# JvanZyl1/PSSO-SAC-for-powered-descent

Hardware: AMD Instinct MI355X
Metric: env-steps/sec at 65 536 parallel envs; achieved HBM GB/s vs peak (higher is better)
Workload: dtype f64; 1 GPU; c3: 65536 envs/GPU, landing_burn_pure_throttle, rtd_rl reward, wind (percentile profile drawn per reset + VK gusts below 15 km) + tilt, auto-reset, uniform random actions; synchronized starts, 640 untimed burn-in + 5 warmup steps; envs_per_gpu=65536, global_envs=65536, parallelism=env-shard x1

## Files before the change

include/pdenv.h:

```cpp
#ifndef PDENV_H
#define PDENV_H
#include <stddef.h>
#include <stdint.h>

#ifdef __cplusplus
extern "C" {
#endif

#define PD_ABI_VERSION 11
#define PD_MAX_PTS 256
#define PD_MAX_COLS 5
#define PD_MAX_TAB 64
#define PD_MAX_WIND 16
#define PD_N_WIND_PROFILES 50
#define PD_N_STATE 11
#define PD_N_INFO 49
#define PD_ACTOR_PARAMS_PURE_THROTTLE 249
#define PD_ACTOR_PARAMS_LANDING_BURN 372

typedef enum { PD_OK = 0, PD_ERR_INVALID = 1, PD_ERR_HIP = 2, PD_ERR_NOMEM = 3, PD_ERR_UNSUPPORTED = 4 } pd_status;
typedef enum {
    PD_PHASE_PURE_THROTTLE = 0, PD_PHASE_LANDING_BURN = 1, PD_PHASE_PCONTROL = 2,
    PD_PHASE_BALLISTIC_ARC = 3, PD_PHASE_FLIP_OVER = 4, PD_PHASE_SUBSONIC = 5, PD_PHASE_SUPERSONIC = 6,
    PD_PHASE_LANDING_BURN_ACS = 7
} pd_phase;
typedef enum { PD_RTD_RL = 0, PD_RTD_PSO = 1, PD_RTD_NONE = 2 } pd_rtd;
typedef enum { PD_F64 = 0, PD_F32 = 1 } pd_precision;
typedef enum { PD_INTEG_REFERENCE = 0, PD_INTEG_RK4 = 1 } pd_integrator;
typedef enum {
    PD_TABLES_NO_CELL_PIECES = 1,
    PD_TABLES_NO_FINE_INDEX = 2,
    PD_TABLES_EXACT_ATMOSPHERE = 4,
    PD_TABLES_VERBOSE = 8
} pd_table_flags;

typedef struct {
    int32_t n_cols, n_pts;
    double col_aoa[PD_MAX_COLS];
    int32_t col_start[PD_MAX_COLS], col_len[PD_MAX_COLS];
    double mach[PD_MAX_PTS];
    double coef[PD_MAX_PTS];
} pd_aero_table;

typedef struct {
    double thrust_per_engine, nozzle_exit_pressure, nozzle_exit_area, v_exhaust;
    int32_t n_engines_gimballed, pad0;
    double grid_fin_area, d_base_grid_fin, rocket_radius, frontal_area, m_prop0, C_gust_x, C_gust_y;
    double h_ox, h_f, m_ox, m_f, h_lower, m_dry, x_dry, I_dry, engine_height, cop;
// ... 145 lines not shown
pd_status pd_set_gload_window(pd_env* env, const void* vprev, const void* window, const uint8_t* len,
                              void* stream);
pd_status pd_get_gload_window(pd_env* env, void* vprev, void* window, uint8_t* len, uint8_t* head, void* stream);
pd_status pd_set_wind_sigmas(pd_env* env, const double* sig, void* stream);
pd_status pd_get_wind_state(pd_env* env, void* filters, void* sigmas, uint8_t* profile, void* stream);
pd_status pd_set_wind_state(pd_env* env, const void* filters, const void* sigmas, const uint8_t* profile, void* stream);
pd_status pd_get_counters(pd_env* env, uint32_t* episode, uint32_t* step, int8_t* trunc_id, void* stream);
pd_status pd_set_counters(pd_env* env, const uint32_t* episode, const uint32_t* step, const int8_t* trunc_id,
                          void* stream);
size_t pd_checkpoint_size(const pd_env* env);
pd_status pd_checkpoint_save(pd_env* env, void* blob, void* stream);
pd_status pd_checkpoint_load(pd_env* env, const void* blob, void* stream);
pd_status pd_counters(pd_env* env, int64_t* rbf_misses, int64_t* table_entries_cd,
                      int64_t* table_entries_cl, int64_t* nan_events);
pd_status pd_atmosphere(pd_env* env, const void* altitude, void* out, int64_t n, void* stream);
#define PD_N_STATS 48
pd_status pd_stats(pd_env* env, int64_t* out, int32_t n);
pd_status pd_count_work(pd_env* env, int32_t enable);
pd_status pd_cell_piece_info(const pd_params* params, int32_t table, int64_t piece, double* out, int32_t n_out);
pd_status pd_atm_table(const pd_params* params, int32_t precision, const double* alt, int64_t n_alt,
                       double* atm_out, double* max_rel);
int pd_obs_dim(const pd_env* env);
int pd_action_dim(const pd_env* env);

#ifdef __cplusplus
}
#endif
#endif
```

psso-sac-for-powered-descent_amd/csrc/pd_physics.h:

```cpp
#pragma once
#include "pd_common.h"

namespace pd {

template <typename R> struct Cst;
template <> struct Cst<double> {
    static constexpr double deg2rad = kDeg2Rad, rad2deg = kRad2Deg, pi = kPi, two_pi = 2 * kPi;
    static constexpr double inf = __builtin_huge_val();
};
template <> struct Cst<float> {
    static constexpr float deg2rad = (float)kDeg2Rad, rad2deg = (float)kRad2Deg, pi = (float)kPi,
                           two_pi = (float)(2 * kPi);
    static constexpr float inf = __builtin_huge_valf();
};

template <typename R> constexpr R veltkamp_c() { return sizeof(R) == 8 ? R(134217729.0) : R(4097.0f); }
template <typename R> constexpr bool one_step_ok(R b, R rb) {
    const R p = b * rb;
    const R C = veltkamp_c<R>();
    const R tb = C * b, bh = tb - (tb - b), bl = b - bh;
    const R tr = C * rb, rh = tr - (tr - rb), rl = rb - rh;
    const R lo = ((bh * rh - p) + bh * rl + bl * rh) + bl * rl;
    const R eps = (p - R(1)) + lo;
    const R lim = sizeof(R) == 8 ? R(0.99 * 0x1p-54) : R(0.99f * 0x1p-25f);
// ... 293 lines not shown
            int j = kind == 5 ? 4 + k : (kind == 6 ? 4 + k : (k < 6 ? k : k + 1));
            put(k, (R)(float)((R)(float)s[j] / P.norm_ph[k]));
        }
    }
}
template <typename R>
__device__ __forceinline__ void obs_write(DP<R>& P, int kind, const R* s, R* out, uint32_t idx) {
    const int d = obs_dim(kind);
    PD_AS1 char* o = (PD_AS1 char*)(uint64_t)out;
    obs_eval<R>(P, kind, s, [&](int k, R v) {
        *(PD_AS1 R*)(o + (uint32_t)(idx * (uint32_t)(d * sizeof(R)) + k * (uint32_t)sizeof(R))) = v;
    });
}

template <typename R>
__device__ __forceinline__ R grid_fin_ca(DP<R>& P, const R* sx, const R* sy, R mach, const uint16_t* lb = nullptr,
                                         const R* slope = nullptr) {
    if (mach < P.ca_min_mach) return P.ca_min_val;
    int n = P.ca_n;
    int lo = 0, hi = n;
    if (lb != nullptr && mach >= R(0) && mach < R(10)) {
        int b = (int)(mach * R(6.4));
        b = b > 63 ? 63 : b;
        const uint32_t rg = lb[b];
        lo = (int)(rg & 0xffu); hi = (int)(rg >> 8);
    }
    while (lo < hi) { int mid = (lo + hi) >> 1; if (sx[mid] < mach) lo = mid + 1; else hi = mid; }
    int idx = lo < 1 ? 1 : (lo > n - 1 ? n - 1 : lo);
    R xl = sx[idx - 1], yl = sy[idx - 1];
    const R sl = slope ? slope[idx] : (sy[idx] - yl) / (sx[idx] - xl);
    return sl * (mach - xl) + yl;
}

template <typename R>
__device__ __forceinline__ R np_interp(const R* x, const R* y, int n, R v, const R* slope = nullptr) {
    if (v < x[0]) return y[0];
    if (v >= x[n - 1]) return y[n - 1];
    int lo = 0, hi = n;
    while (lo < hi) { int mid = (lo + hi) >> 1; if (x[mid] <= v) lo = mid + 1; else hi = mid; }
    int j = lo - 1;
    if (x[j] == v) return y[j];
    const R sl = slope ? slope[j] : (y[j + 1] - y[j]) / (x[j + 1] - x[j]);
    return sl * (v - x[j]) + y[j];
}

template <typename R>
__device__ __forceinline__ R grid_fin_cn_alpha(DP<R>& P, const R* sx, const R* sy, R mach, const R* slope = nullptr) {
    if (mach < P.cn_min_mach) return P.cn_min_val;
    if (mach <= P.cn_max_mach) return np_interp(sx, sy, P.cn_n, mach, slope);
    return P.cn_max_val + P.cn_slope * (mach - P.cn_max_mach);
}

template <typename R> struct RbfCache {
    unsigned long long key;
    int slot;
};

template <typename R>
// ... 65 lines not shown
```

psso-sac-for-powered-descent_amd/csrc/pd_step.h:

```cpp
#pragma once
#include <hip/hip_runtime.h>

#include <cstring>

#include "../../include/pdenv.h"
#include "pd_physics.h"
#include "pd_sac_mlp.h"

namespace pd {

constexpr int kBlock = 256;
constexpr int kStepBlock = 256;
constexpr int kScratch = kSys * kSys + kSys + 3 * kNbr + kPay;
constexpr int kPendingCap = 4096;
constexpr int kSolveSlots = 1024;
constexpr int kGridExact = 1 << 30;
constexpr int kGridRefine = 1 << 29;
constexpr int kGridBisect = 1 << 28;
constexpr int kGridPiece = 1 << 27;
constexpr uint32_t kFinePiece = 1u << 30;
constexpr uint32_t kFineBisect = 1u << 29;
constexpr uint32_t kFineRefined = 1u << 28;
constexpr uint32_t kFineIndex = kFineRefined - 1u;

// ... 2 lines not shown
constexpr int kCellExact = 4;
constexpr int kCellKey = kCellCoef + 3 * kCellExact;
constexpr int kCellStride = (kCellKey + 2) & ~1;
constexpr int kCellKeyF = (kCellKey + 1) & ~1;
constexpr int kCellStrideF = (kCellKeyF + 2 + 3) & ~3;
template <typename R> constexpr int cell_stride() { return sizeof(R) == 8 ? kCellStride : kCellStrideF; }
template <typename R> constexpr int cell_key() { return sizeof(R) == 8 ? kCellKey : kCellKeyF; }

struct GridBisect {
    double nx, ny, c, tau;
    unsigned long long key_a, key_b;
    int slot_a, slot_b;
    int piece_a, piece_b;
};
constexpr int kGridSub = 8;
constexpr int kStats = 48;

enum Stat {
    kStMisses = 0, kStNan = 1, kStInsCd = 2, kStInsCl = 3,
    kStStamp = 8,
    kStDropped = 16,
    kStWork = 32,
    kStGust = kStWork + 0,
    kStResets = kStWork + 1,
    kStQLine = kStWork + 2,
    kStQVerify = kStWork + 3,
    kStQTaylor = kStWork + 4,
    kStQBal = kStWork + 5,
    kStQMiss = kStWork + 6,
    kStBalRounds = kStWork + 7,
    kStQRefined = kStWork + 8,
    kStQBisect = kStWork + 9,
    kStWRefined = kStWork + 10,
    kStWBisect = kStWork + 11,
    kStQCell = kStWork + 12,
    kStWMixed = kStWork + 13,
    kNWork = 14
};

struct WaveCount {
    uint32_t* w;
    __device__ __forceinline__ void add(int k, bool pred) {
        if (w) {
            const uint32_t v = (uint32_t)__popcll(__ballot(pred));
            if (__lane_id() == 0) w[k] += v;
        }
    }
    __device__ __forceinline__ void add_n(int k, uint32_t v) {
        if (w && __lane_id() == 0) w[k] += v;
    }
};

template <typename R> struct LineLds {
    R bp[4][kLineMax];
    int slot[4][kLineMax + 1];
    unsigned long long key[4][kLineMax + 1];
    R a[4];
    int nbp[4];
    int tay_off[4];
    uint16_t lb[4][kLineBuckets];
};

template <typename R, bool WIND> struct alignas(16) StepStatic {
    alignas(16) R tab[1024];
// ... 79 lines not shown
        for (uint32_t p = 0; p <= mask; ++p) {
            const unsigned long long k = keys[h];
            if (k == key) { slot = -1; break; }
            if (k == kEmptyKey) { slot = (int)h; break; }
            h = (h + 1) & mask;
        }
        if (slot >= 0 && stats[kStInsCd + table] * 2 + 2 > (1ull << lc)) slot = -1;
        if (slot < 0) continue;
        stats[kStInsCd + table] += 1;
        keys[slot] = key;
        pay_store<R>(ppay + e * kPay, (table ? pay_cl : pay_cd) + (int64_t)slot * pay_stride<R>());
    }
    *count = 0;
}

template <typename R> struct StepArgs {
    uint64_t P;
    EnvBufs<R> b;
    Pending pend;
    int64_t n;
    uint64_t env_offset;
    uint32_t seed_lo, seed_hi;
    int act_f64, auto_reset, stochastic, fixed_prof, use_tilt;
    double tilt_sigma;
    const void* actions;
    R* obs; R* reward; uint8_t* done; uint8_t* trunc; int8_t* trunc_id;
    const double* noise;
    R* info;
    uint64_t info_mask;
    int info_nsel;
// ... 37 lines not shown
```

psso-sac-for-powered-descent_amd/csrc/pd_step_impl.h:

```cpp
#pragma once
#include "pd_envdev.h"

namespace pd {

__device__ __forceinline__ int dpp_swap1(int v) { return __builtin_amdgcn_mov_dpp(v, 0xB1, 0xF, 0xF, false); }
__device__ __forceinline__ float pair_swap(float v) { return __int_as_float(dpp_swap1(__float_as_int(v))); }
__device__ __forceinline__ double pair_swap(double v) {
    const uint64_t b = (uint64_t)__double_as_longlong(v);
    const uint32_t lo = (uint32_t)dpp_swap1((int)(uint32_t)b), hi = (uint32_t)dpp_swap1((int)(uint32_t)(b >> 32));
    return __longlong_as_double((long long)(((uint64_t)hi << 32) | lo));
}

template <int LPE, typename R>
__device__ __forceinline__ void sincos_pair(R x0, R x1, int role, R& s0, R& c0, R& s1, R& c1) {
    if constexpr (LPE >= 2) {
        const bool odd = role & 1;
        R s, c;
        pd_sincos<R>(odd ? x1 : x0, s, c);
        const R so = pair_swap(s), co = pair_swap(c);
        s0 = odd ? so : s; c0 = odd ? co : c;
        s1 = odd ? s : so; c1 = odd ? c : co;
    } else {
        pd_sincos<R>(x0, s0, c0);
        pd_sincos<R>(x1, s1, c1);
// ... 820 lines not shown
    if constexpr (OSPLIT) gather(ys, y, OS);
    else {
#pragma unroll
        for (int j = 0; j < OUT; ++j) y[j] = ys[j];
    }
}

#ifdef PD_STAMP
#define PD_T(v) const unsigned long long v = __builtin_amdgcn_s_memtime()
#define PD_ACC(k, d) acc_[k] += (d)
#else
#define PD_T(v)
#define PD_ACC(k, d)
#endif

template <typename R, bool WIND, int EPB, bool BAL = false> struct StepLds : StepStatic<R, WIND> {
    R gwin[10][EPB];
    uint32_t work[kStepBlock / 64][kNWork];
    double wnx[WIND ? 2 : 1][WIND ? kStepBlock : 1];
    BalLds<R> bal[BAL ? kStepBlock / 64 : 1];
    TabView<R> tdesc[2];
};

template <typename R>
__device__ __forceinline__ TabView<R> tab_view_lds(const TabView<R>* d, int table) { return d[table]; }
template <typename R>
__device__ __forceinline__ TabView<R> tab_view(DP<R>& P, const R* tab, int table) {
    TabView<R> t;
    t.smach = tab + (table ? 512 : 0);
    t.start = table ? &P.cl_start[0] : &P.cd_start[0];
    t.n = table ? &P.cl_len[0] : &P.cd_len[0];
    t.aoa = table ? &P.cl_aoa[0] : &P.cd_aoa[0];
    t.keys = gbl(table ? P.keys_cl : P.keys_cd);
// ... 12 lines not shown
    t.grid_na = P.grid_na[table];
    t.grid_a0 = P.grid_a0[table];
    t.grid_inv_da = P.grid_inv_da[table];
    t.grid_inv_dm = P.grid_inv_dm[table];
    return t;
}

template <typename R, int PHASE, int RTD, bool WIND, int LPE, int POL = 0, bool RK4 = false, bool CNT = false,
          bool SAC = false, bool ROLL = false>
__global__ __launch_bounds__(kStepBlock) __attribute__((amdgpu_waves_per_eu(2))) void k_step(StepArgs<R> a_) {
    SA<R>& a = kargs<R>();
    static_assert(sizeof(a_) > 0);
    static_assert(!ROLL || (SAC && LPE == 16 && !POL && !RK4 && !CNT && RTD == 0 && PHASE <= 1),
                  "ROLL: the SAC kernel of the RL landing burns at 16 lanes per env");
    constexpr int EPB = kStepBlock / LPE;
    __shared__ StepLds<R, WIND, EPB, LPE == 2> L;
#ifdef PD_STAMP
    unsigned long long acc_[17] = {};
#endif
    PD_T(t_start);
    int64_t n_act = a.n;
    constexpr bool kRefill = POL && !WIND;
    int64_t ring_pos0 = 0;
    if constexpr (SAC) { if (a.ring_state) ring_pos0 = (int64_t)__atomic_load_n(a.ring_state, __ATOMIC_RELAXED); }
    if constexpr (POL) {
        if (blockIdx.x == 0 && threadIdx.x == 0) *a.cnt_zero = 0u;
        if (kRefill && a.refill) n_act = a.refill_slots;
        if (a.use_list) {
            n_act = (int64_t)*a.cnt_in;
            if ((int64_t)blockIdx.x * EPB >= n_act) return;
        }
// ... 18 lines not shown
    const int le = (int)threadIdx.x / LPE;
    uint32_t ui = (uint32_t)i;
    bool live = valid;
    if constexpr (POL) {
        if (!a.use_list) live = live && ev(a.b.fin, ui) == 0;
    }
    if constexpr (ROLL) live = live && ev(a.b.fin, ui) == 0;
    constexpr int nparts = LPE >= 2 ? LPE / 2 : 1;
    const int my_table = LPE >= 2 ? role / nparts : 0;
    const int part = LPE >= 2 ? role % nparts : 0;
    const int gbase = (int)__lane_id() & ~(LPE - 1);
    uint64_t g = a.env_offset + (uint64_t)i;

    EnvRegs<R> e;
    RbfCache<R> cA, cB;
    auto load_env = [&]() {
        DP<R>& P = *params<R>(a.P);
#pragma unroll
        for (int k = 0; k < 11; ++k) e.s[k] = valid ? ldv(a.b.st + (k) * N, ui) : P.state0[k];
        e.vprev = valid ? ldv(a.b.vprev, ui) : sqrt(e.s[2] * e.s[2] + e.s[3] * e.s[3]);
        e.glen = valid ? (int)ldv(a.b.glen, ui) : 0;
        e.ghead = valid ? (int)ldv(a.b.ghead, ui) : 0;
#pragma unroll
        for (int k = 0; k < 10; ++k) L.gwin[k][le] = valid ? ldv(a.b.gwin + (k) * N, ui) : R(0);
        e.act0 = R(0); e.act1 = R(0); e.act2 = R(0);
        if constexpr (PHASE == 1 || PHASE == 2) e.act0 = valid ? ldv(a.b.act, ui) : R(0);
        if constexpr (PHASE == 1) {
            e.act1 = valid ? ldv(a.b.act + N, ui) : R(0);
            e.act2 = valid ? ldv(a.b.act + (2) * N, ui) : R(0);
        }
        e.fu0 = R(0); e.fu1 = R(0); e.fv0 = R(0); e.fv1 = R(0); e.sgu = R(0); e.sgv = R(0); e.prof = 0;
        if constexpr (WIND) {
            if (valid) {
                e.fu0 = ldv(a.b.wind, ui); e.fu1 = ldv(a.b.wind + N, ui);
                e.fv0 = ldv(a.b.wind + (2) * N, ui); e.fv1 = ldv(a.b.wind + (3) * N, ui);
                e.sgu = ldv(a.b.wind + (4) * N, ui); e.sgv = ldv(a.b.wind + (5) * N, ui);
                e.prof = ldv(a.b.wprof, ui);
            }
        }
        e.ep = valid ? ldv(a.b.epi, ui) : 0u;
        e.ts = valid ? ldv(a.b.tstep, ui) : 0u;
        e.tid = valid ? (int)ldv(a.b.tid, ui) : 0;
        cA.key = valid ? ldv(a.b.key + (my_table) * N, ui) : (my_table ? P.init_key_cl : P.init_key_cd);
        cA.slot = valid ? ldv(a.b.slot + (my_table) * N, ui) : -1;
        if constexpr (LPE == 1) { cB.key = valid ? ldv(a.b.key + N, ui) : P.init_key_cl; cB.slot = valid ? ldv(a.b.slot + N, ui) : -1; }
        else { cB.key = 0; cB.slot = -1; }
    };
    load_env();
    constexpr int kImg = (int)(sizeof(StepStatic<R, WIND>) / 16);
    constexpr int kLog = (int)(sizeof(LogTableD) / 16);
    constexpr int kPer = (kImg + kLog + kStepBlock - 1) / kStepBlock;
    using V4 = __attribute__((ext_vector_type(4))) unsigned int;
    V4 stg[kPer];
    {
        DP<R>& P = *params<R>(a.P);
        const PD_AS1 V4* img = (const PD_AS1 V4*)P.stage_img;
        const PD_AS1 V4* lgt = (const PD_AS1 V4*)(uint64_t)&P.logtab_d.cell[0];
#pragma unroll
        for (int k = 0; k < kPer; ++k) {
// ... 16 lines not shown
                if (a.sac_heads_out && e0 + e < a.n) a.sac_heads_out[(e0 + e) * 2 * A2 + o] = v;
            };
            if (H == 128) sac_mlp_tile<128>(a.sac_mlp, a.n, e0, s_mlp, put);
            else sac_mlp_tile<256>(a.sac_mlp, a.n, e0, s_mlp, put);
            __syncthreads();
        }
    }
    {
        DP<R>& P = *params<R>(a.P);
#pragma unroll
        for (int k = 0; k < kPer; ++k) {
            const int t = threadIdx.x + k * kStepBlock;
            if (t < kImg) ((V4*)static_cast<StepStatic<R, WIND>*>(&L))[t] = stg[k];
            else if (t < kImg + kLog) ((V4*)s_logtab)[t - kImg] = stg[k];
        }
        if (threadIdx.x < (kStepBlock / 64) * kNWork) (&L.work[0][0])[threadIdx.x] = 0u;
        if (threadIdx.x < 2) L.tdesc[threadIdx.x] = tab_view<R>(P, L.tab, (int)threadIdx.x);
    }
    __syncthreads();
    PD_T(t_staged);
    PD_ACC(0, t_staged - t_start);
    if constexpr (POL) {
        if (!a.use_list && __ballot(live) == 0) return;
    }
    const int aux = PHASE == 2 ? params<R>(a.P)->phase : PHASE;
    const bool ascent = PHASE == 2 && (aux == PD_PHASE_SUBSONIC || aux == PD_PHASE_SUPERSONIC);
    constexpr int A = PHASE == 0 ? 1 : (PHASE == 1 ? 4 : 2);
    const int AD = PHASE == 2 ? (ascent ? 2 : 1) : A;
    static_assert(!RK4 || (PHASE == 0 && !WIND && !POL), "RK4: pure throttle, no wind, no policy");
    constexpr int NSUB = RK4 ? 40 : (PHASE == 2 ? 1 : 4);
    constexpr bool kAtmTab = sizeof(R) == 4 || !WIND;
    constexpr bool kPcs = !WIND && !RK4 && LPE <= 8 && (PHASE == 0 || (PHASE == 1 && !SAC));
    const R dt = RK4 ? R(0.01) : (PHASE == 0 ? R(0.025) : (PHASE == 1 ? R(0.1) : (R)a.dt_aux));
    const R dt_act = PHASE == 2 ? dt : R(0.025);
    PD_T(t_loaded);
    PD_ACC(1, t_loaded - t_staged);

    auto store_all = [&]() {
    uint32_t uo = ui;
    asm volatile("" : "+v"(uo));
    if (live) {
        const uint32_t ui = uo;
#pragma unroll
        for (int k = 0; k < 11; ++k)
            if (k % LPE == role) ev(a.b.st + (k) * N, ui) = e.s[k];
// ... 43 lines not shown
        if (a.roll_steps) ev(a.roll_steps, uo) = (int32_t)steps;
        if (a.roll_done) ev(a.roll_done, uo) = (uint8_t)dn_;
        if (a.roll_tid) ev(a.roll_tid, uo) = (int8_t)id_;
        if (fin_) ev(a.b.fin, uo) = 1;
    };
    WaveCount wc{CNT ? L.work[threadIdx.x >> 6] : nullptr};
    R k_rho = R(0), k_patm = R(0), k_asnd = R(0);
    double k_speed = 0.0;
    bool k_have = false;
    using RS = double;
    RS xs[sizeof(R) == 8 ? 1 : 11];
    auto SV = [&](int k) -> RS& {
        if constexpr (sizeof(R) == 8) return e.s[k];
        else return xs[k];
    };
#pragma unroll 1
    for (int f = 0; f < nf; ++f) {
    SA<R>& a = kargs<R>();
    const size_t fo = (size_t)f * (size_t)N;
    float uf[A];
    double ud[A];
#pragma unroll
    for (int k = 0; k < A; ++k) { uf[k] = 0.f; ud[k] = 0.0; }
    if constexpr (ROLL) {
        if (role == 0) {
            DP<R>& Q = *params<R>(a.P);
            constexpr int ok = PHASE == 0 ? 0 : 3;
            obs_eval<R>(Q, ok, e.s, [&](int k, R v) { s_obs[le * obs_dim(ok) + k] = (float)v; });
        }
        if (!__syncthreads_or(live ? 1 : 0)) break;
// ... 42 lines not shown
            float xk = m;
            if (a.sac_eps || a.sac_draw) {
                float ls = mlp ? s_sach[le * 16 + 8 + k] : ldv(a.sac_logstd + k, ui * a.sac_hs);
                ls = ls < a.sac_lo ? a.sac_lo : (ls > a.sac_hi ? a.sac_hi : ls);
                const float sd = expf(ls);
                const float ek = a.sac_draw ? ed[k] : ldv(a.sac_eps + k, ui * AD);
                xk = m + sd * ek;
                if (a.sac_eps_out && role == 0 && live) ev(a.sac_eps_out + k, ui * AD) = ek;
            }
            uf[k] = tanhf(xk) * a.sac_max;
            if (a.sac_act && role == 0 && live) ev(a.sac_act + k, ui * AD) = uf[k];
            if constexpr (ROLL) {
                if (a.roll_act && role == 0 && live)
                    ev(a.roll_act + (size_t)(a.roll_t0 + f) * (size_t)N * (size_t)AD + k, ui * AD) = uf[k];
            }
        }
    } else if (a.act_f64) {
#pragma unroll
        for (int k = 0; k < A; ++k) if (k < AD) ud[k] = ldv((const double*)a.actions + fo * AD + k, ui * AD);
    } else {
#pragma unroll
        for (int k = 0; k < A; ++k) if (k < AD) uf[k] = ldv((const float*)a.actions + fo * AD + k, ui * AD);
    }
    constexpr int kObsKind = RTD == 1 ? (PHASE == 0 ? 1 : 2) : (PHASE == 0 ? 0 : (PHASE == 1 ? 3 : -1));
    uint32_t srow = ui;
    if (SAC && a.ring_state) {
        const int64_t rp = ring_pos0 + (int64_t)i;
        srow = (uint32_t)(rp >= a.ring_cap ? rp - a.ring_cap : rp);
    }
    if (SAC && a.slab && role == 0 && live) {
// ... 20 lines not shown

    bool wpre = false;
    RS rkb[8], rka[8];
    if constexpr (sizeof(R) == 4) {
#pragma unroll
        for (int k = 0; k < 11; ++k) xs[k] = (RS)e.s[k];
    }
    const RS dts = RK4 ? 0.01 : (PHASE == 0 ? 0.025 : (PHASE == 1 ? 0.1 : a.dt_aux));
#pragma unroll 1
    for (int sub = 0; sub < NSUB; ++sub) {
        PD_T(t_sub);
        const int stage = RK4 ? (sub & 3) : 0;
        SA<R>& a = kargs<R>();
        DP<R>& P = *params<R>(a.P);
        const bool tap_sub = tap && sub == NSUB - 1;
        RS x = SV(0), y = SV(1), vx = SV(2), vy = SV(3), th = SV(4), thd = SV(5), ga = SV(6), al = SV(7);
        RS m = SV(8), mp = SV(9);
        if constexpr (WIND) wc.add(kStGust - kStWork, role == 0 && live && a.stochastic && y < P.vk_y_threshold);
        R rho, patm, asnd;
        RS speed;
        if (RK4 ? (sub == 0 && k_have) : k_have) { rho = k_rho; patm = k_patm; asnd = k_asnd; speed = k_speed; }
        else {
            atmosphere<R, kAtmTab>(P, L.isa, (R)y, rho, patm, asnd);
            speed = sqrt(vx * vx + vy * vy);
        }
        const R spR = (R)speed;
        R mach = R(0);
        if (asnd != R(0)) { R mr = spR / asnd; mach = (R(10) < mr) ? R(10) : mr; }
        const R ae = (R)((vy < RS(0)) ? ga - th - Cst<RS>::pi : al);
        R ug = R(0), vg = R(0);
        auto wind_block = [&]() {
            if constexpr (WIND) {
                const R* walt = L.walt + e.prof * 16;
                const R* wsp = L.wsp + e.prof * 16;
                R km = PD_DIVC(R, (R)y, 1000);
                int wn = P.wind_n[e.prof];
                ug = np_interp<R>(walt, wsp, wn, km);
                const bool gust = y < P.vk_y_threshold && a.stochastic;
                if (gust) {
                    double w0 = 0.0, w1 = 0.0;
                    const double* lic = (const double*)(uint64_t)&P.logtab.invc[0];
                    const double* llc = (const double*)(uint64_t)&P.logtab.logc[0];
                    bool drawn = false;
                    if (a.noise) { w0 = ev(a.noise + 2 * sub, ui * 8); w1 = ev(a.noise + 2 * sub + 1, ui * 8); drawn = true; }
                    else if constexpr (LPE >= 2 && NSUB == 4) {
                        if ((sub & 1) == 0) {
                            const int odd = role & 1;
                            u32x4 r = philox_k({(uint32_t)g, (uint32_t)(g >> 32) ^ e.ep, e.ts, kTagWindSub + (uint32_t)(sub + odd)},
                                             a.seed_lo, a.seed_hi);
                            double z0, z1;
                            gauss_pair(r, lic, llc, z0, z1);
                            const double o0 = pair_swap(z0), o1 = pair_swap(z1);
// ... 92 lines not shown
        R sae, cae, sth, cth;
        sincos_pair<LPE, R>(ae, (R)th, role, sae, cae, sth, cth);
        R apar, aperp;
        if (vy >= RS(0)) { apar = lift * sae - drag * cae; aperp = -lift * cae - drag * sae; }
        else { apar = drag * cae - lift * sae; aperp = -drag * sae - lift * cae; }
        R aero_x = apar * cth + aperp * sth;
        R aero_y = apar * sth - aperp * cth;
        R aero_m = aperp * d_cp_cg;
        if (PHASE == 2 && aux == PD_PHASE_FLIP_OVER) { aero_x = R(0); aero_y = R(0); aero_m = R(0); }

#ifdef PD_STAMP
        PD_T(t_p2); acc_[9 + 5] += t_p2 - t_p1;
#endif
        R T_full = P.T_e + (P.p_e - patm) * P.A_e;
        R qS = q * P.S_gf;
        R Ca = grid_fin_ca<R>(P, L.gf, L.gf + 64, mach, L.ca_lb, L.gfs);
        R cfp, cfperp, cm, mdot_dt, md_info, thr_info;
        R i_dl = R(0), i_dr = R(0), i_cnl = R(0), i_cnr = R(0), i_gfperp = R(0), i_gfpar = R(0), i_gfm = R(0);
        bool f32_forces = false;
        float cfp_f = 0.f, cfperp_f = 0.f;
        if constexpr (PHASE == 2) {
            if (aux == PD_PHASE_PCONTROL) {
                R u0;
                if (a.act_f64) {
                    R nt = ((R)ud[0] - spR) * P.kp_pc;
                    nt = nt < R(0) ? R(0) : (nt > R(1) ? R(1) : nt);
                    u0 = R(2) * (nt - R(0.5));
                } else {
                    float nt = (uf[0] - (float)speed) * P.f_kp_pc;
                    nt = nt < 0.f ? 0.f : (nt > 1.f ? 1.f : nt);
                    u0 = (R)(2.0f * (nt - 0.5f));
// ... 200 lines not shown
        if (ga < RS(0)) ga = Cst<RS>::two_pi + ga;
        al = th - ga;
        mp -= (RS)mdot_dt; m -= (RS)mdot_dt;
        }
        if (tap_sub) {
            info(PD_INFO_CF_X, cfx); info(PD_INFO_CF_Y, cfy); info(PD_INFO_GRAVITY, gr); info(PD_INFO_VX_DOT, vxd);
            info(PD_INFO_VY_DOT, vyd); info(PD_INFO_MOMENTS, mz); info(PD_INFO_THETA_DDOT, thdd);
        }
        SV(0) = x; SV(1) = y; SV(2) = vx; SV(3) = vy; SV(4) = th; SV(5) = thd; SV(6) = ga; SV(7) = al;
        SV(8) = m; SV(9) = mp;
        if (!RK4 || stage == 3) SV(10) = SV(10) + dts;
        PD_T(t_subend);
        PD_ACC(4, t_subend - t_aero1);
    }
    if (nan_hit && role == 0 && live) atomicAdd(&a.pend.stats[kStNan], 1ull);
    if constexpr (sizeof(R) == 4) {
#pragma unroll
        for (int k = 0; k < 11; ++k) e.s[k] = (R)xs[k];
    }
    PD_T(t_loop);

    DP<R>& P2 = *params<R>(a.P);
    const R* s = e.s;
    const RS v = RK4 ? sqrt(SV(2) * SV(2) + SV(3) * SV(3)) : k_speed;
    R gl_new = (R)PD_DIVC(RS, PD_DIVC(RS, fabs(v - (RS)e.vprev), 0.1) * RS(1), 9.81);
    int glen = e.glen, ghead = e.ghead;
    int wslot;
    if (glen < 10) { wslot = glen; glen += 1; }
    else { wslot = ghead; ghead = ghead == 9 ? 0 : ghead + 1; }
    L.gwin[wslot][le] = gl_new;
// ... 315 lines not shown
#pragma unroll
        for (int k = 0; k < 7; ++k) atomicAdd(&a.pend.stats[kStStamp + k], acc_[k]);
        atomicAdd(&a.pend.stats[kStStamp + 7], 1ull);
        atomicAdd(&a.pend.stats[22], acc_[7]);
        atomicAdd(&a.pend.stats[23], acc_[8]);
        for (int k = 0; k < 4; ++k) atomicAdd(&a.pend.stats[24 + k], acc_[9 + k]);
        for (int k = 0; k < 4; ++k) atomicAdd(&a.pend.stats[28 + k], acc_[13 + k]);
    }
#endif
}

template <typename R, int PH, int RT, bool W, int LPE, bool RK> void launch_step(const StepArgs<R>& a, hipStream_t s) {
    unsigned grid = (unsigned)((a.n * LPE + kStepBlock - 1) / kStepBlock);
    const bool sac = a.sac_mean != nullptr || a.sac_mlp.H != 0;
    if constexpr (LPE == 2 && !RK) {
        if (a.count_work && !sac) {
            hipLaunchKernelGGL((k_step<R, PH, RT, W, LPE, 0, RK, true>), dim3(grid), dim3(kStepBlock), 0, s, a);
            return;
        }
    }
    if constexpr (RT == 0 && PH <= 1 && !RK) {
        if (sac) {
            hipLaunchKernelGGL((k_step<R, PH, RT, W, LPE, 0, RK, false, true>), dim3(grid), dim3(kStepBlock), 0, s, a);
            return;
        }
    }
    if (sac) return;
    hipLaunchKernelGGL((k_step<R, PH, RT, W, LPE, 0, RK>), dim3(grid), dim3(kStepBlock), 0, s, a);
}

template <typename R, int PH, bool W, int LPE> void launch_policy_lpe(const StepArgs<R>& a, int64_t n_launch,
// ... 12 lines not shown
```

psso-sac-for-powered-descent_amd/csrc/pdenv.hip:

```cpp
#include <hip/hip_runtime.h>

#include <algorithm>
#include <array>
#include <chrono>
#include <cmath>
#include <cstdio>
#include <cstdlib>
#include <cstring>
#include <map>
#include <mutex>
#include <string>
#include <thread>
#include <vector>

#include "../../include/pdenv.h"
#include "pd_envdev.h"

using namespace pd;

namespace pd {
thread_local std::string g_err;
pd_status set_error(pd_status s, const char* m) { g_err = m; return s; }
}

// ... 1159 lines not shown
    a.b.act = (R*)e->act; a.b.wind = (R*)e->wind; a.b.wprof = e->wprof; a.b.key = e->key; a.b.slot = e->slot;
    a.b.tid = e->tid; a.b.epi = e->epi; a.b.tstep = e->tstep; a.b.fin = e->fin;
    a.pend = e->pend;
    a.n = e->cfg.n_envs;
    a.env_offset = e->cfg.env_offset;
    a.seed_lo = (uint32_t)e->cfg.seed; a.seed_hi = (uint32_t)(e->cfg.seed >> 32);
    a.act_f64 = e->cfg.action_f64;
    a.auto_reset = e->cfg.auto_reset;
    a.stochastic = e->cfg.stochastic_wind;
    a.fixed_prof = e->cfg.wind_percentile >= 50 ? e->cfg.wind_percentile - 50 : -1;
    a.use_tilt = e->cfg.tilt_sigma_rad > 0.0;
    a.tilt_sigma = e->cfg.tilt_sigma_rad;
    a.dt_aux = e->cfg.dt > 0.0 ? e->cfg.dt : 0.1;
    a.rtd_none = e->cfg.rtd == PD_RTD_NONE;
    a.n_fused = 1;
    a.count_work = e->count_work;
    return a;
}

template <typename R> void fill_params(const pd_params* p, const pd_config* c, DevParams<R>& D) {
    std::memset(&D, 0, sizeof(D));
    D.T_e = (R)p->thrust_per_engine; D.p_e = (R)p->nozzle_exit_pressure; D.A_e = (R)p->nozzle_exit_area;
    D.v_ex = (R)p->v_exhaust; D.S_gf = (R)p->grid_fin_area; D.d_base_gf = (R)p->d_base_grid_fin;
    D.R_rocket = (R)p->rocket_radius; D.A_front = (R)p->frontal_area; D.m_prop0 = (R)p->m_prop0;
    D.C_gust_x = (R)p->C_gust_x; D.C_gust_y = (R)p->C_gust_y; D.n_eng = p->n_engines_gimballed;
    double nom_pt = (0 * 0.4) / (double)p->n_engines_gimballed;
    double nom_lb = (3 * 0.4) / (double)p->n_engines_gimballed;
    double te_vex = p->thrust_per_engine / p->v_exhaust;
    double mg = 5.0 * kDeg2Rad, md = 20.0 * kDeg2Rad;
    D.f_Te_over_vex = (float)te_vex; D.f_one_minus_nom_pt = (float)(1 - nom_pt); D.f_nom_pt = (float)nom_pt;
    D.f_one_minus_nom_lb = (float)(1 - nom_lb); D.f_nom_lb = (float)nom_lb; D.f_dt_pt = (float)0.025;
// ... 105 lines not shown
                                        "base_environment.py:150); use PD_RTD_NONE for physics stepping");
    if (c->rtd == PD_RTD_PSO && c->phase > PD_PHASE_LANDING_BURN)
        return fail(PD_ERR_UNSUPPORTED, "rtd PSO exists for the two landing burns only: the other rtd_pso functions take "
                                        "(state) / (state, done, truncated) and raise TypeError when the env calls them "
                                        "(rtd_pso.py:38,63,107,120,141,157 vs base_environment.py:150-152)");
    if (c->dt < 0.0) return fail(PD_ERR_INVALID, "dt must be >= 0");
    if (c->rtd == PD_RTD_RL && (c->phase == PD_PHASE_LANDING_BURN || c->phase == PD_PHASE_PCONTROL) &&
        (c->trajectory_length < 1 || !(c->discount_factor > 0.0 && c->discount_factor < 1.0)))
        return fail(PD_ERR_INVALID, "this RL reward needs discount_factor in (0, 1) and trajectory_length >= 1");
    if (c->phase == PD_PHASE_SUBSONIC || c->phase == PD_PHASE_SUPERSONIC) {
        if (!p->ref_y || !p->ref_x || !p->ref_vx || !p->ref_vy || p->n_ref < 2)
            return fail(PD_ERR_INVALID, "ascent phases need the reference trajectory (ref_y/x/vx/vy, n_ref >= 2)");
    }
    if (c->precision != PD_F64 && c->precision != PD_F32) return fail(PD_ERR_INVALID, "bad precision");
    if (c->integrator != PD_INTEG_REFERENCE && c->integrator != PD_INTEG_RK4) return fail(PD_ERR_INVALID, "bad integrator");
    if (c->table_flags & ~(PD_TABLES_NO_CELL_PIECES | PD_TABLES_NO_FINE_INDEX | PD_TABLES_EXACT_ATMOSPHERE | PD_TABLES_VERBOSE))
        return fail(PD_ERR_INVALID, "unknown table_flags bits");
    if (c->integrator == PD_INTEG_RK4 && (c->phase != PD_PHASE_PURE_THROTTLE || c->enable_wind))
        return fail(PD_ERR_UNSUPPORTED, "the RK4 integrator (non-parity, BASELINE c2) exists for "
                                        "landing_burn_pure_throttle without wind only");
    for (const pd_aero_table* t : {&p->cd, &p->cl})
        for (int k = 0; k < t->n_cols; ++k)
            if (!(t->col_aoa[k] >= 0.0 && t->col_aoa[k] <= 255.0 && t->col_aoa[k] == (double)(int)t->col_aoa[k]))
                return fail(PD_ERR_INVALID, "aero table column AoAs must be integers in [0, 255]");
    if (c->action_f64 && c->precision != PD_F64) return fail(PD_ERR_INVALID, "f64 actions need PD_F64");
    if (c->enable_wind && !(c->wind_percentile == -1 || (c->wind_percentile >= 50 && c->wind_percentile <= 99)))
        return fail(PD_ERR_INVALID, "wind_percentile must be 50..99 or -1");
    const pd_aero_table* ts[2] = {&p->cd, &p->cl};
    for (auto t : ts) {
        if (t->n_cols != kCols || t->n_pts < kNbr || t->n_pts > PD_MAX_PTS) return fail(PD_ERR_INVALID, "aero table shape");
        int s = 0;
// ... 1084 lines not shown
```

psso-sac-for-powered-descent_amd/pdenv/_lib.py:

```python
import ctypes as C
import os

HERE = os.path.dirname(os.path.abspath(__file__))
LIB_PATH = os.path.join(HERE, "libpdenv.so")

D, I32, I64, U64 = C.c_double, C.c_int32, C.c_int64, C.c_uint64
MAX_PTS, MAX_COLS, MAX_TAB, MAX_WIND, N_PROF = 256, 5, 64, 16, 50
N_STATE, N_INFO = 11, 49

PD_OK, PD_ERR_INVALID, PD_ERR_HIP, PD_ERR_NOMEM, PD_ERR_UNSUPPORTED = range(5)
(PURE_THROTTLE, LANDING_BURN, PCONTROL, BALLISTIC_ARC, FLIP_OVER, SUBSONIC, SUPERSONIC,
 LANDING_BURN_ACS) = range(8)
RTD_RL, RTD_PSO, RTD_NONE = 0, 1, 2
F64, F32 = 0, 1
ACTOR_PARAMS = {0: 249, 1: 372}

INFO_FIELDS = ["air_density", "atmospheric_pressure", "speed_of_sound", "mach_number",
               "dynamic_pressure", "CL", "CD", "mass_flow", "x_cog", "inertia",
               "alpha_effective", "throttle", "g_load_1_sec_window", "ug", "vg", "gimbal_angle_deg",
               "mach_number_max", "drag", "lift", "d_cp_cg", "d_thrust_cg", "fuel_percentage_consumed",
               "control_force_parallel", "control_force_perpendicular", "control_force_x", "control_force_y",
               "aero_force_x", "aero_force_y", "gravity", "F_wind_x", "F_wind_y", "vx_dot", "vy_dot",
               "control_moment_z", "aero_moment_z", "M_wind_z", "moments_z", "theta_dot_dot",
               "delta_command_left_rad", "delta_command_right_rad", "delta_left_rad", "delta_right_rad",
# ... 36 lines not shown
        ("ref_y", C.POINTER(D)), ("ref_x", C.POINTER(D)), ("ref_vx", C.POINTER(D)), ("ref_vy", C.POINTER(D)),
        ("n_ref", I32), ("pad2", I32),
        ("hyper", ((D * 9) * 12) * 2), ("terminal_mach", D * 2),
    ]


class PdConfig(C.Structure):
    _fields_ = [("n_envs", I64), ("device", I32), ("phase", I32), ("rtd", I32), ("precision", I32),
                ("seed", U64), ("env_offset", U64), ("enable_wind", I32), ("stochastic_wind", I32),
                ("wind_percentile", I32), ("auto_reset", I32), ("tilt_sigma_rad", D),
                ("action_f64", I32), ("lanes_per_env", I32),
                ("dt", D), ("discount_factor", D), ("trajectory_length", I32), ("integrator", I32),
                ("table_flags", I32), ("pad3", I32)]


TABLES_NO_CELL_PIECES, TABLES_NO_FINE_INDEX, TABLES_EXACT_ATMOSPHERE, TABLES_VERBOSE = 1, 2, 4, 8


class PdTuning(C.Structure):
    _fields_ = [("step_fuse", I32), ("policy_fuse", I32), ("policy_lanes", I32), ("policy_list", I32),
                ("policy_list_at", D), ("policy_refill", I32), ("policy_slots", I32),
                ("policy_refill_own", I32), ("pad_tuning", I32)]


EXPORTS = ["pd_abi_version", "pd_sizeof_params", "pd_sizeof_config", "pd_last_error", "pd_device_count", "pd_create",
           "pd_destroy", "pd_reset", "pd_step", "pd_step_n", "pd_rollout", "pd_rollout_policy", "pd_pso_step",
           "pd_flush_misses", "pd_observe", "pd_get_state", "pd_set_state", "pd_get_actuators", "pd_set_actuators",
           "pd_set_gload_window", "pd_get_gload_window", "pd_set_wind_sigmas", "pd_get_wind_state",
           "pd_set_wind_state", "pd_get_counters", "pd_set_counters", "pd_checkpoint_size", "pd_checkpoint_save",
           "pd_checkpoint_load", "pd_counters", "pd_stats", "pd_count_work", "pd_atmosphere", "pd_obs_dim",
           "pd_action_dim", "pd_step_sac", "pd_pso_swarm_minima", "pd_pso_update_bests", "pd_cell_piece_info",
# ... 103 lines not shown
```

psso-sac-for-powered-descent_amd/pdenv/env.py:

```python
import ctypes as C

import torch

from . import _lib as L
from .params import Params

PHASES = {"landing_burn_pure_throttle": L.PURE_THROTTLE, "landing_burn": L.LANDING_BURN,
          "landing_burn_pure_throttle_Pcontrol": L.PCONTROL, "ballistic_arc_descent": L.BALLISTIC_ARC,
          "flip_over_boostbackburn": L.FLIP_OVER, "subsonic": L.SUBSONIC, "supersonic": L.SUPERSONIC,
          "landing_burn_ACS": L.LANDING_BURN_ACS}
MODES = {"rl": L.RTD_RL, "pso": L.RTD_PSO, "physics": L.RTD_NONE}
INTEGRATORS = {"reference": 0, "rk4": 1}
UNSTEPPABLE = {("landing_burn_ACS", m) for m in MODES} | {("flip_over_boostbackburn", "rl")} | \
    {(p, "pso") for p in PHASES if p not in ("landing_burn_pure_throttle", "landing_burn")}


def _stream(device):
    return C.c_void_p(torch.cuda.current_stream(device).cuda_stream)


def _ptr(t):
    return None if t is None else C.c_void_p(t.data_ptr())


# ... 361 lines not shown
        tid = torch.empty(self.n, dtype=torch.int8, **kw)
        L.check(self.lib.pd_get_counters(self.h, _ptr(ep), _ptr(st), _ptr(tid), _stream(self.device)))
        return ep, st, tid

    def atmosphere(self, altitude):
        alt = torch.as_tensor(altitude, dtype=self.dtype).to(self.device).reshape(-1).contiguous()
        out = torch.empty(3, alt.numel(), dtype=self.dtype, device=self.device)
        L.check(self.lib.pd_atmosphere(self.h, _ptr(alt), _ptr(out), int(alt.numel()), _stream(self.device)))
        return out[0], out[1], out[2]

    def count_work(self, enable=True):
        L.check(self.lib.pd_count_work(self.h, int(bool(enable))))

    WORK_COUNTERS = ("gust_substeps", "resets", "q_line", "q_verified", "q_taylor", "q_balanced", "q_miss",
                     "balanced_rounds", "q_refined", "q_bisect", "wave_substeps_refined", "wave_substeps_bisect",
                     "q_cell", "wave_substeps_mixed")

    def stats(self):
        v = (L.I64 * 48)()
        L.check(self.lib.pd_stats(self.h, v, 48))
        out = {"rbf_misses": v[0], "nan_events": v[1], "table_entries_cd": v[2], "table_entries_cl": v[3],
               "miss_queue_dropped": v[16]}
        out.update({k: v[32 + j] for j, k in enumerate(self.WORK_COUNTERS)})
        return out

    def counters(self):
        v = [L.I64() for _ in range(4)]
        L.check(self.lib.pd_counters(self.h, *[C.byref(x) for x in v]))
        return {"rbf_misses": v[0].value, "table_entries_cd": v[1].value, "table_entries_cl": v[2].value,
                "nan_events": v[3].value}

    def close(self):
        if getattr(self, "h", None):
            self.lib.pd_destroy(self.h)
            self.h = None
# ... 7 lines not shown
```

Baseline: 2.169 billion env-steps/s.

## Carry table-search indices across substeps and prefetch next frame's actions

Adds a per-thread packed carry word that remembers the last bracket index for the wind-profile interpolation and the grid-fin Ca table. Each substep first checks the remembered bracket and falls back to binary search only when it misses, which removes most search iterations and LDS loads. Separately, when there is no policy and no SAC, the next frame's actions are loaded at the end of each frame so the global-load latency overlaps other work. It also shrinks the LDS work-counter array when counting is off. The cost is extra registers and some divergence on carry misses, plus a new flag and counters to disable the carry or measure hit rates.

```diff
diff --git a/include/pdenv.h b/include/pdenv.h
--- a/include/pdenv.h
+++ b/include/pdenv.h
@@ -31,7 +31,8 @@
     PD_TABLES_NO_CELL_PIECES = 1,
     PD_TABLES_NO_FINE_INDEX = 2,
     PD_TABLES_EXACT_ATMOSPHERE = 4,
-    PD_TABLES_VERBOSE = 8
+    PD_TABLES_VERBOSE = 8,
+    PD_TABLES_NO_CARRY = 16
 } pd_table_flags;
 
 typedef struct {
@@ -207,7 +208,7 @@
 pd_status pd_counters(pd_env* env, int64_t* rbf_misses, int64_t* table_entries_cd,
                       int64_t* table_entries_cl, int64_t* nan_events);
 pd_status pd_atmosphere(pd_env* env, const void* altitude, void* out, int64_t n, void* stream);
-#define PD_N_STATS 48
+#define PD_N_STATS 64
 pd_status pd_stats(pd_env* env, int64_t* out, int32_t n);
 pd_status pd_count_work(pd_env* env, int32_t enable);
 pd_status pd_cell_piece_info(const pd_params* params, int32_t table, int64_t piece, double* out, int32_t n_out);
diff --git a/psso-sac-for-powered-descent_amd/csrc/pd_physics.h b/psso-sac-for-powered-descent_amd/csrc/pd_physics.h
--- a/psso-sac-for-powered-descent_amd/csrc/pd_physics.h
+++ b/psso-sac-for-powered-descent_amd/csrc/pd_physics.h
@@ -331,10 +331,7 @@
 }
 
 template <typename R>
-__device__ __forceinline__ R grid_fin_ca(DP<R>& P, const R* sx, const R* sy, R mach, const uint16_t* lb = nullptr,
-                                         const R* slope = nullptr) {
-    if (mach < P.ca_min_mach) return P.ca_min_val;
-    int n = P.ca_n;
+__device__ __forceinline__ int grid_fin_ca_search(const R* sx, int n, R mach, const uint16_t* lb) {
     int lo = 0, hi = n;
     if (lb != nullptr && mach >= R(0) && mach < R(10)) {
         int b = (int)(mach * R(6.4));
@@ -343,22 +340,89 @@
         lo = (int)(rg & 0xffu); hi = (int)(rg >> 8);
     }
     while (lo < hi) { int mid = (lo + hi) >> 1; if (sx[mid] < mach) lo = mid + 1; else hi = mid; }
+    return lo;
+}
+template <typename R>
+__device__ __forceinline__ R grid_fin_ca(DP<R>& P, const R* sx, const R* sy, R mach, const uint16_t* lb = nullptr,
+                                         const R* slope = nullptr) {
+    if (mach < P.ca_min_mach) return P.ca_min_val;
+    int n = P.ca_n;
+    const int lo = grid_fin_ca_search<R>(sx, n, mach, lb);
     int idx = lo < 1 ? 1 : (lo > n - 1 ? n - 1 : lo);
     R xl = sx[idx - 1], yl = sy[idx - 1];
     const R sl = slope ? slope[idx] : (sy[idx] - yl) / (sx[idx] - xl);
     return sl * (mach - xl) + yl;
 }
 
+#ifndef PD_CARRY
+#define PD_CARRY 7
+#endif
+constexpr uint32_t kCarryWindShift = 0, kCarryWindMask = 0xfu, kCarryFinShift = 4, kCarryFinMask = 0xffu;
+constexpr uint32_t kCarryNone = 0xffffffffu;
+__device__ __forceinline__ uint32_t carry_get(uint32_t cw, uint32_t shift, uint32_t mask) { return (cw >> shift) & mask; }
+__device__ __forceinline__ uint32_t carry_set(uint32_t cw, uint32_t shift, uint32_t mask, uint32_t v) {
+    return (cw & ~(mask << shift)) | ((v & mask) << shift);
+}
+enum CarryRes { kCarrySkip = 0, kCarryHit = 1, kCarrySearch = 2 };
+
+template <typename R>
+__device__ __forceinline__ R grid_fin_ca_carry(DP<R>& P, const R* sx, const R* sy, R mach, const uint16_t* lb,
+                                               const R* slope, uint32_t& g, int& res) {
+    res = kCarrySkip;
+    if (mach < P.ca_min_mach) return P.ca_min_val;
+    const int n = P.ca_n;
+    bool ok = g != kCarryFinMask && (int)g <= n;
+    int lo = ok ? (int)g : 0;
+    int idx = lo < 1 ? 1 : (lo > n - 1 ? n - 1 : lo);
+    const R xa = sx[lo > 0 ? lo - 1 : 0], xb = sx[lo < n ? lo : n - 1];
+    R xl = sx[idx - 1], yl = sy[idx - 1];
+    R sl = slope[idx];
+    ok = ok && (lo == 0 || xa < mach) && (lo == n || xb >= mach);
+    res = ok ? kCarryHit : kCarrySearch;
+    if (!ok) {
+        lo = grid_fin_ca_search<R>(sx, n, mach, lb);
+        idx = lo < 1 ? 1 : (lo > n - 1 ? n - 1 : lo);
+        xl = sx[idx - 1]; yl = sy[idx - 1];
+        sl = slope[idx];
+    }
+    g = (uint32_t)lo;
+    return sl * (mach - xl) + yl;
+}
+
+template <typename R>
+__device__ __forceinline__ int np_interp_search(const R* x, int n, R v) {
+    int lo = 0, hi = n;
+    while (lo < hi) { int mid = (lo + hi) >> 1; if (x[mid] <= v) lo = mid + 1; else hi = mid; }
+    return lo - 1;
+}
 template <typename R>
 __device__ __forceinline__ R np_interp(const R* x, const R* y, int n, R v, const R* slope = nullptr) {
     if (v < x[0]) return y[0];
     if (v >= x[n - 1]) return y[n - 1];
-    int lo = 0, hi = n;
-    while (lo < hi) { int mid = (lo + hi) >> 1; if (x[mid] <= v) lo = mid + 1; else hi = mid; }
-    int j = lo - 1;
+    int j = np_interp_search<R>(x, n, v);
     if (x[j] == v) return y[j];
     const R sl = slope ? slope[j] : (y[j + 1] - y[j]) / (x[j + 1] - x[j]);
     return sl * (v - x[j]) + y[j];
+}
+
+template <typename R>
+__device__ __forceinline__ R np_interp_carry(const R* x, const R* y, int n, R v, uint32_t& g, int& res) {
+    bool ok = g != kCarryWindMask && (int)g < n - 1;
+    int j = ok ? (int)g : 0;
+    R x0 = x[j], x1 = x[j + 1], y0 = y[j], y1 = y[j + 1];
+    ok = ok && x0 <= v && v < x1;
+    res = ok ? kCarryHit : kCarrySearch;
+    if (!ok) {
+        res = kCarrySkip;
+        if (v < x[0]) return y[0];
+        if (v >= x[n - 1]) return y[n - 1];
+        res = kCarrySearch;
+        j = np_interp_search<R>(x, n, v);
+        x0 = x[j]; y0 = y[j]; x1 = x[j + 1]; y1 = y[j + 1];
+        g = (uint32_t)j;
+    }
+    if (x0 == v) return y0;
+    return (y1 - y0) / (x1 - x0) * (v - x0) + y0;
 }
 
 template <typename R>
diff --git a/psso-sac-for-powered-descent_amd/csrc/pd_step.h b/psso-sac-for-powered-descent_amd/csrc/pd_step.h
--- a/psso-sac-for-powered-descent_amd/csrc/pd_step.h
+++ b/psso-sac-for-powered-descent_amd/csrc/pd_step.h
@@ -40,7 +40,7 @@
     int piece_a, piece_b;
 };
 constexpr int kGridSub = 8;
-constexpr int kStats = 48;
+constexpr int kStats = 64;
 
 enum Stat {
     kStMisses = 0, kStNan = 1, kStInsCd = 2, kStInsCl = 3,
@@ -61,7 +61,9 @@
     kStWBisect = kStWork + 11,
     kStQCell = kStWork + 12,
     kStWMixed = kStWork + 13,
-    kNWork = 14
+    kStCWindHit = kStWork + 14, kStCWindSearch = kStWork + 15,
+    kStCFinHit = kStWork + 16, kStCFinSearch = kStWork + 17,
+    kNWork = 18
 };
 
 struct WaveCount {
@@ -74,6 +76,12 @@
     }
     __device__ __forceinline__ void add_n(int k, uint32_t v) {
         if (w && __lane_id() == 0) w[k] += v;
+    }
+    __device__ __forceinline__ void add_carry(int k, bool hit, bool search) {
+        if (w) {
+            const bool s = __ballot(search) != 0ull, h = __ballot(hit) != 0ull;
+            if (__lane_id() == 0) { w[k] += (uint32_t)(h && !s); w[k + 1] += (uint32_t)s; }
+        }
     }
 };
 
@@ -183,6 +191,7 @@
     *count = 0;
 }
 
+constexpr int kArgCount = 1, kArgNoCarry = 2;
 template <typename R> struct StepArgs {
     uint64_t P;
     EnvBufs<R> b;
diff --git a/psso-sac-for-powered-descent_amd/csrc/pd_step_impl.h b/psso-sac-for-powered-descent_amd/csrc/pd_step_impl.h
--- a/psso-sac-for-powered-descent_amd/csrc/pd_step_impl.h
+++ b/psso-sac-for-powered-descent_amd/csrc/pd_step_impl.h
@@ -858,9 +858,9 @@
 #define PD_ACC(k, d)
 #endif
 
-template <typename R, bool WIND, int EPB, bool BAL = false> struct StepLds : StepStatic<R, WIND> {
+template <typename R, bool WIND, int EPB, bool BAL = false, bool CNT = false> struct StepLds : StepStatic<R, WIND> {
     R gwin[10][EPB];
-    uint32_t work[kStepBlock / 64][kNWork];
+    uint32_t work[kStepBlock / 64][CNT ? kNWork : 1];
     double wnx[WIND ? 2 : 1][WIND ? kStepBlock : 1];
     BalLds<R> bal[BAL ? kStepBlock / 64 : 1];
     TabView<R> tdesc[2];
@@ -903,7 +903,7 @@
     static_assert(!ROLL || (SAC && LPE == 16 && !POL && !RK4 && !CNT && RTD == 0 && PHASE <= 1),
                   "ROLL: the SAC kernel of the RL landing burns at 16 lanes per env");
     constexpr int EPB = kStepBlock / LPE;
-    __shared__ StepLds<R, WIND, EPB, LPE == 2> L;
+    __shared__ StepLds<R, WIND, EPB, LPE == 2, CNT> L;
 #ifdef PD_STAMP
     unsigned long long acc_[17] = {};
 #endif
@@ -952,6 +952,7 @@
 
     EnvRegs<R> e;
     RbfCache<R> cA, cB;
+    uint32_t carry;
     auto load_env = [&]() {
         DP<R>& P = *params<R>(a.P);
 #pragma unroll
@@ -981,6 +982,7 @@
         e.tid = valid ? (int)ldv(a.b.tid, ui) : 0;
         cA.key = valid ? ldv(a.b.key + (my_table) * N, ui) : (my_table ? P.init_key_cl : P.init_key_cd);
         cA.slot = valid ? ldv(a.b.slot + (my_table) * N, ui) : -1;
+        carry = kCarryNone;
         if constexpr (LPE == 1) { cB.key = valid ? ldv(a.b.key + N, ui) : P.init_key_cl; cB.slot = valid ? ldv(a.b.slot + N, ui) : -1; }
         else { cB.key = 0; cB.slot = -1; }
     };
@@ -1027,7 +1029,7 @@
             if (t < kImg) ((V4*)static_cast<StepStatic<R, WIND>*>(&L))[t] = stg[k];
             else if (t < kImg + kLog) ((V4*)s_logtab)[t - kImg] = stg[k];
         }
-        if (threadIdx.x < (kStepBlock / 64) * kNWork) (&L.work[0][0])[threadIdx.x] = 0u;
+        if constexpr (CNT) { if (threadIdx.x < (kStepBlock / 64) * kNWork) (&L.work[0][0])[threadIdx.x] = 0u; }
         if (threadIdx.x < 2) L.tdesc[threadIdx.x] = tab_view<R>(P, L.tab, (int)threadIdx.x);
     }
     __syncthreads();
@@ -1042,6 +1044,13 @@
     const int AD = PHASE == 2 ? (ascent ? 2 : 1) : A;
     static_assert(!RK4 || (PHASE == 0 && !WIND && !POL), "RK4: pure throttle, no wind, no policy");
     constexpr int NSUB = RK4 ? 40 : (PHASE == 2 ? 1 : 4);
+#ifndef PD_CARRY_WIDE
+#define PD_CARRY_WIDE 0
+#endif
+    constexpr bool kSpills = RK4 && LPE == 16;
+    constexpr bool kCarry = (PD_CARRY & 3) != 0 && (PD_CARRY_WIDE || (sizeof(R) == 8 && !kSpills && !SAC));
+    constexpr bool kActAhead = (PD_CARRY & 4) != 0 && !POL && !SAC &&
+                               (PD_CARRY_WIDE || (PHASE == 0 && sizeof(R) == 8 && !kSpills));
     constexpr bool kAtmTab = sizeof(R) == 4 || !WIND;
     constexpr bool kPcs = !WIND && !RK4 && LPE <= 8 && (PHASE == 0 || (PHASE == 1 && !SAC));
     const R dt = RK4 ? R(0.01) : (PHASE == 0 ? R(0.025) : (PHASE == 1 ? R(0.1) : (R)a.dt_aux));
@@ -1115,6 +1124,29 @@
         if constexpr (sizeof(R) == 8) return e.s[k];
         else return xs[k];
     };
+    uint32_t an0[kActAhead ? A : 1], an1[kActAhead ? A : 1];
+    auto act_request = [&](int fr) {
+        if constexpr (kActAhead) {
+            SA<R>& a = kargs<R>();
+            const size_t fo = (size_t)fr * (size_t)N;
+            if (a.act_f64) {
+#pragma unroll
+                for (int k = 0; k < A; ++k) if (k < AD) {
+                    const unsigned long long w = (unsigned long long)__double_as_longlong(
+                        ldv((const double*)a.actions + fo * AD + k, ui * AD));
+                    an0[k] = (uint32_t)w; an1[k] = (uint32_t)(w >> 32);
+                }
+            } else {
+#pragma unroll
+                for (int k = 0; k < A; ++k) if (k < AD) an0[k] = __float_as_uint(ldv((const float*)a.actions + fo * AD + k, ui * AD));
+            }
+        }
+    };
+    if constexpr (kActAhead) {
+#pragma unroll
+        for (int k = 0; k < A; ++k) { an0[k] = 0u; an1[k] = 0u; }
+        if (nf > 0) act_request(0);
+    }
 #pragma unroll 1
     for (int f = 0; f < nf; ++f) {
     SA<R>& a = kargs<R>();
@@ -1187,6 +1219,12 @@
                 if (a.roll_act && role == 0 && live)
                     ev(a.roll_act + (size_t)(a.roll_t0 + f) * (size_t)N * (size_t)AD + k, ui * AD) = uf[k];
             }
+        }
+    } else if constexpr (kActAhead) {
+#pragma unroll
+        for (int k = 0; k < A; ++k) if (k < AD) {
+            if (a.act_f64) ud[k] = __longlong_as_double((long long)(((unsigned long long)an1[k] << 32) | an0[k]));
+            else uf[k] = __uint_as_float(an0[k]);
         }
     } else if (a.act_f64) {
 #pragma unroll
@@ -1237,6 +1275,7 @@
         SA<R>& a = kargs<R>();
         DP<R>& P = *params<R>(a.P);
         const bool tap_sub = tap && sub == NSUB - 1;
+        if constexpr (kCarry) { if (a.count_work & kArgNoCarry) carry = kCarryNone; }
         RS x = SV(0), y = SV(1), vx = SV(2), vy = SV(3), th = SV(4), thd = SV(5), ga = SV(6), al = SV(7);
         RS m = SV(8), mp = SV(9);
         if constexpr (WIND) wc.add(kStGust - kStWork, role == 0 && live && a.stochastic && y < P.vk_y_threshold);
@@ -1258,7 +1297,15 @@
                 const R* wsp = L.wsp + e.prof * 16;
                 R km = PD_DIVC(R, (R)y, 1000);
                 int wn = P.wind_n[e.prof];
-                ug = np_interp<R>(walt, wsp, wn, km);
+                if constexpr (kCarry && (PD_CARRY & 1)) {
+                    uint32_t wj = carry_get(carry, kCarryWindShift, kCarryWindMask);
+                    int wres;
+                    ug = np_interp_carry<R>(walt, wsp, wn, km, wj, wres);
+                    carry = carry_set(carry, kCarryWindShift, kCarryWindMask, wj);
+                    wc.add_carry(kStCWindHit - kStWork, live && wres == kCarryHit, live && wres == kCarrySearch);
+                } else {
+                    ug = np_interp<R>(walt, wsp, wn, km);
+                }
                 const bool gust = y < P.vk_y_threshold && a.stochastic;
                 if (gust) {
                     double w0 = 0.0, w1 = 0.0;
@@ -1381,7 +1428,16 @@
 #endif
         R T_full = P.T_e + (P.p_e - patm) * P.A_e;
         R qS = q * P.S_gf;
-        R Ca = grid_fin_ca<R>(P, L.gf, L.gf + 64, mach, L.ca_lb, L.gfs);
+        R Ca;
+        if constexpr (kCarry && (PD_CARRY & 2)) {
+            uint32_t fg = carry_get(carry, kCarryFinShift, kCarryFinMask);
+            int fres;
+            Ca = grid_fin_ca_carry<R>(P, L.gf, L.gf + 64, mach, L.ca_lb, L.gfs, fg, fres);
+            carry = carry_set(carry, kCarryFinShift, kCarryFinMask, fg);
+            wc.add_carry(kStCFinHit - kStWork, live && fres == kCarryHit, live && fres == kCarrySearch);
+        } else {
+            Ca = grid_fin_ca<R>(P, L.gf, L.gf + 64, mach, L.ca_lb, L.gfs);
+        }
         R cfp, cfperp, cm, mdot_dt, md_info, thr_info;
         R i_dl = R(0), i_dr = R(0), i_cnl = R(0), i_cnr = R(0), i_gfperp = R(0), i_gfpar = R(0), i_gfm = R(0);
         bool f32_forces = false;
@@ -1612,6 +1668,7 @@
         PD_ACC(4, t_subend - t_aero1);
     }
     if (nan_hit && role == 0 && live) atomicAdd(&a.pend.stats[kStNan], 1ull);
+    if constexpr (kActAhead) { if (f + 1 < nf) act_request(f + 1); }
     if constexpr (sizeof(R) == 4) {
 #pragma unroll
         for (int k = 0; k < 11; ++k) e.s[k] = (R)xs[k];
@@ -1957,7 +2014,7 @@
     unsigned grid = (unsigned)((a.n * LPE + kStepBlock - 1) / kStepBlock);
     const bool sac = a.sac_mean != nullptr || a.sac_mlp.H != 0;
     if constexpr (LPE == 2 && !RK) {
-        if (a.count_work && !sac) {
+        if ((a.count_work & kArgCount) && !sac) {
             hipLaunchKernelGGL((k_step<R, PH, RT, W, LPE, 0, RK, true>), dim3(grid), dim3(kStepBlock), 0, s, a);
             return;
         }
diff --git a/psso-sac-for-powered-descent_amd/csrc/pdenv.hip b/psso-sac-for-powered-descent_amd/csrc/pdenv.hip
--- a/psso-sac-for-powered-descent_amd/csrc/pdenv.hip
+++ b/psso-sac-for-powered-descent_amd/csrc/pdenv.hip
@@ -1197,7 +1197,7 @@
     a.dt_aux = e->cfg.dt > 0.0 ? e->cfg.dt : 0.1;
     a.rtd_none = e->cfg.rtd == PD_RTD_NONE;
     a.n_fused = 1;
-    a.count_work = e->count_work;
+    a.count_work = (e->count_work ? kArgCount : 0) | ((e->cfg.table_flags & PD_TABLES_NO_CARRY) ? kArgNoCarry : 0);
     return a;
 }
 
@@ -1333,7 +1333,8 @@
     }
     if (c->precision != PD_F64 && c->precision != PD_F32) return fail(PD_ERR_INVALID, "bad precision");
     if (c->integrator != PD_INTEG_REFERENCE && c->integrator != PD_INTEG_RK4) return fail(PD_ERR_INVALID, "bad integrator");
-    if (c->table_flags & ~(PD_TABLES_NO_CELL_PIECES | PD_TABLES_NO_FINE_INDEX | PD_TABLES_EXACT_ATMOSPHERE | PD_TABLES_VERBOSE))
+    if (c->table_flags & ~(PD_TABLES_NO_CELL_PIECES | PD_TABLES_NO_FINE_INDEX | PD_TABLES_EXACT_ATMOSPHERE | PD_TABLES_VERBOSE |
+                           PD_TABLES_NO_CARRY))
         return fail(PD_ERR_INVALID, "unknown table_flags bits");
     if (c->integrator == PD_INTEG_RK4 && (c->phase != PD_PHASE_PURE_THROTTLE || c->enable_wind))
         return fail(PD_ERR_UNSUPPORTED, "the RK4 integrator (non-parity, BASELINE c2) exists for "
diff --git a/psso-sac-for-powered-descent_amd/pdenv/_lib.py b/psso-sac-for-powered-descent_amd/pdenv/_lib.py
--- a/psso-sac-for-powered-descent_amd/pdenv/_lib.py
+++ b/psso-sac-for-powered-descent_amd/pdenv/_lib.py
@@ -74,7 +74,7 @@
                 ("table_flags", I32), ("pad3", I32)]
 
 
-TABLES_NO_CELL_PIECES, TABLES_NO_FINE_INDEX, TABLES_EXACT_ATMOSPHERE, TABLES_VERBOSE = 1, 2, 4, 8
+TABLES_NO_CELL_PIECES, TABLES_NO_FINE_INDEX, TABLES_EXACT_ATMOSPHERE, TABLES_VERBOSE, TABLES_NO_CARRY = 1, 2, 4, 8, 16
 
 
 class PdTuning(C.Structure):
diff --git a/psso-sac-for-powered-descent_amd/pdenv/env.py b/psso-sac-for-powered-descent_amd/pdenv/env.py
--- a/psso-sac-for-powered-descent_amd/pdenv/env.py
+++ b/psso-sac-for-powered-descent_amd/pdenv/env.py
@@ -399,11 +399,12 @@
 
     WORK_COUNTERS = ("gust_substeps", "resets", "q_line", "q_verified", "q_taylor", "q_balanced", "q_miss",
                      "balanced_rounds", "q_refined", "q_bisect", "wave_substeps_refined", "wave_substeps_bisect",
-                     "q_cell", "wave_substeps_mixed")
+                     "q_cell", "wave_substeps_mixed",
+                     "carry_wind_hit", "carry_wind_search", "carry_fin_hit", "carry_fin_search")
 
     def stats(self):
-        v = (L.I64 * 48)()
-        L.check(self.lib.pd_stats(self.h, v, 48))
+        v = (L.I64 * 64)()
+        L.check(self.lib.pd_stats(self.h, v, 64))
         out = {"rbf_misses": v[0], "nan_events": v[1], "table_entries_cd": v[2], "table_entries_cl": v[3],
                "miss_queue_dropped": v[16]}
         out.update({k: v[32 + j] for j, k in enumerate(self.WORK_COUNTERS)})
```

New measurement: 2.233 billion env-steps/s, median of 6. 1.03x the previous value.
